# Dustin-Ray/capyCRYPT

Measured on NVIDIA B200. Metric: sha3_256_GBps, higher is better.
Workload: dtype u64

## Files before the change

### capycrypt_b200/csrc/keccak_bs.cuh

```cuda
#pragma once
#include <cstdint>

#include "keccak.cuh"

namespace capy {

static __device__ const uint2 KECCAK_RC_BITS[32] = {
    {0x50F4F1u, 0x0DB916u}, {0x000000u, 0x8C7F94u}, {0x000000u, 0x000000u}, {0x000000u, 0x327356u},
    {0x000000u, 0x000000u}, {0x000000u, 0x000000u}, {0x000000u, 0x000000u}, {0x000000u, 0xB5D4DEu},
    {0x000000u, 0x000000u}, {0x000000u, 0x000000u}, {0x000000u, 0x000000u}, {0x000000u, 0x000000u},
    {0x000000u, 0x000000u}, {0x000000u, 0x000000u}, {0x000000u, 0x000000u}, {0x000000u, 0xD81C68u},
    {0x000000u, 0x000000u}, {0x000000u, 0x000000u}, {0x000000u, 0x000000u}, {0x000000u, 0x000000u},
    {0x000000u, 0x000000u}, {0x000000u, 0x000000u}, {0x000000u, 0x000000u}, {0x000000u, 0x000000u},
    {0x000000u, 0x000000u}, {0x000000u, 0x000000u}, {0x000000u, 0x000000u}, {0x000000u, 0x000000u},
    {0x000000u, 0x000000u}, {0x000000u, 0x000000u}, {0x000000u, 0x000000u}, {0x000000u, 0xBBE0CCu}};

template <int K>
__device__ __forceinline__ uint32_t bs_from(uint32_t v, uint32_t lane) {
  if constexpr (K % 32 == 0) return v;
  else return __shfl_sync(0xffffffffu, v, (int)(lane - (uint32_t)K));
}

template <int R>
__device__ __forceinline__ void bs_rot(uint32_t (&b)[2], uint32_t t0, uint32_t t1, uint32_t lane) {
  if constexpr (R % 2 == 0) {
    b[0] = bs_from<R / 2>(t0, lane);
    b[1] = bs_from<R / 2>(t1, lane);
  } else {
    b[0] = bs_from<(R + 1) / 2>(t1, lane);
    b[1] = bs_from<(R - 1) / 2>(t0, lane);
  }
}

#define CAPY_BS_RHO_PI(X, Y, R)                                                                       \
  bs_rot<(R)>(b[(Y) + 5 * ((2 * (X) + 3 * (Y)) % 5)],                                                 \
              lop_xor3(a[(X) + 5 * (Y)][0], c[((X) + 4) % 5][0], n[((X) + 1) % 5][0]),                \
              lop_xor3(a[(X) + 5 * (Y)][1], c[((X) + 4) % 5][1], n[((X) + 1) % 5][1]), lane);

__device__ __forceinline__ uint32_t bs_flip_if(uint32_t v, uint32_t rounds, uint32_t round) {
  asm("{\n\t.reg .pred p;\n\t.reg .b32 t;\n\tand.b32 t, %1, %2;\n\tsetp.ne.u32 p, t, 0;\n\t@p not.b32 %0, %0;\n\t}"
      : "+r"(v)
      : "r"(rounds), "r"(round));
  return v;
}

__device__ __forceinline__ void keccak_bs_round(uint32_t (&a)[25][2], uint32_t lane, uint2 rc, uint32_t round) {
  uint32_t c[5][2], n[5][2], b[25][2];
#pragma unroll
  for (int x = 0; x < 5; x++) {
#pragma unroll
    for (int h = 0; h < 2; h++) c[x][h] = lop_xor3(lop_xor3(a[x][h], a[x + 5][h], a[x + 10][h]), a[x + 15][h], a[x + 20][h]);
    n[x][0] = bs_from<1>(c[x][1], lane);
    n[x][1] = c[x][0];
  }
  CAPY_BS_RHO_PI(0, 0, 0)  CAPY_BS_RHO_PI(1, 0, 1)  CAPY_BS_RHO_PI(2, 0, 62) CAPY_BS_RHO_PI(3, 0, 28) CAPY_BS_RHO_PI(4, 0, 27)
  CAPY_BS_RHO_PI(0, 1, 36) CAPY_BS_RHO_PI(1, 1, 44) CAPY_BS_RHO_PI(2, 1, 6)  CAPY_BS_RHO_PI(3, 1, 55) CAPY_BS_RHO_PI(4, 1, 20)
  CAPY_BS_RHO_PI(0, 2, 3)  CAPY_BS_RHO_PI(1, 2, 10) CAPY_BS_RHO_PI(2, 2, 43) CAPY_BS_RHO_PI(3, 2, 25) CAPY_BS_RHO_PI(4, 2, 39)
  CAPY_BS_RHO_PI(0, 3, 41) CAPY_BS_RHO_PI(1, 3, 45) CAPY_BS_RHO_PI(2, 3, 15) CAPY_BS_RHO_PI(3, 3, 21) CAPY_BS_RHO_PI(4, 3, 8)
  CAPY_BS_RHO_PI(0, 4, 18) CAPY_BS_RHO_PI(1, 4, 2)  CAPY_BS_RHO_PI(2, 4, 61) CAPY_BS_RHO_PI(3, 4, 56) CAPY_BS_RHO_PI(4, 4, 14)
#pragma unroll
  for (int y = 0; y < 5; y++) {
#pragma unroll
    for (int x = 0; x < 5; x++) {
#pragma unroll
      for (int h = 0; h < 2; h++)
        a[x + 5 * y][h] = lop_chi(b[x + 5 * y][h], b[(x + 1) % 5 + 5 * y][h], b[(x + 2) % 5 + 5 * y][h]);
    }
  }
  a[0][0] = bs_flip_if(a[0][0], rc.x, round);
  a[0][1] = bs_flip_if(a[0][1], rc.y, round);
}
#undef CAPY_BS_RHO_PI

struct BsTranspose {
  uint32_t rot[5], keep[5];
  __device__ __forceinline__ explicit BsTranspose(uint32_t lane) {
#pragma unroll
    for (int k = 0; k < 5; k++) {
      const uint32_t d = 16u >> k;
      const uint32_t lo_bits = k == 0 ? 0x0000FFFFu : k == 1 ? 0x00FF00FFu : k == 2 ? 0x0F0F0F0Fu : k == 3 ? 0x33333333u : 0x55555555u;
      const bool upper = lane & d;
      rot[k] = upper ? 32u - d : d;
      keep[k] = upper ? ~lo_bits : lo_bits;
    }
  }
  __device__ __forceinline__ uint32_t operator()(uint32_t x) const {
#pragma unroll
    for (int k = 0; k < 5; k++) {
      const uint32_t y = __shfl_xor_sync(0xffffffffu, x, 16u >> k);
      const uint32_t r = __funnelshift_l(y, y, rot[k]);
      asm("lop3.b32 %0, %0, %1, %2, 0xE4;" : "+r"(x) : "r"(r), "r"(keep[k]));
    }
    return x;
  }
};

__device__ __forceinline__ void bs_gather(uint32_t (&w)[2], uint32_t lo, uint32_t hi, uint32_t lane) {
#pragma unroll
  for (int h = 0; h < 2; h++) {
    const int src = (int)(2 * lane + h);
    const uint32_t l = __shfl_sync(0xffffffffu, lo, src);
    const uint32_t u = __shfl_sync(0xffffffffu, hi, src);
    w[h] = lane < 16 ? l : u;
  }
}

__device__ __forceinline__ void bs_scatter(uint32_t& lo, uint32_t& hi, const uint32_t (&w)[2], uint32_t lane) {
  const int src = (int)(lane >> 1);
  const uint32_t l0 = __shfl_sync(0xffffffffu, w[0], src), l1 = __shfl_sync(0xffffffffu, w[1], src);
  const uint32_t u0 = __shfl_sync(0xffffffffu, w[0], src + 16), u1 = __shfl_sync(0xffffffffu, w[1], src + 16);
  lo = lane & 1 ? l1 : l0;
  hi = lane & 1 ? u1 : u0;
}

}
```

### capycrypt_b200/csrc/sha3_api.cu

```cuda
#include <algorithm>
#include <cmath>
#include <cstdlib>
#include <memory>
#include <thread>
#include <type_traits>
#include <vector>

#include "internal.h"
#include "hostbatch.h"
#include "keccak_bs.cuh"
#include "sponge.cuh"

namespace capy {

template <int LANES>
__global__ void __launch_bounds__(128)
    sha3_uniform_kernel(const uint8_t* __restrict__ data, uint64_t stride, uint64_t len, uint32_t suffix,
                        uint8_t* __restrict__ out, uint32_t out_bytes, uint64_t n) {
  const uint64_t i = (uint64_t)blockIdx.x * blockDim.x + threadIdx.x;
  if (i >= n) return;
  constexpr uint64_t RATE = 8ull * LANES;
  const uint2* q = reinterpret_cast<const uint2*>(data + i * stride);
  Lane a[25];
  state_zero(a);
  const uint64_t nfull = len / RATE;
  for (uint64_t b = 0; b < nfull; b++) {
#pragma unroll
    for (int j = 0; j < LANES; j++) {
      uint2 v = __ldg(q + j);
      a[j].lo ^= v.x;
      a[j].hi ^= v.y;
    }
    q += LANES;
    keccak_f1600(a);
  }
  const uint32_t rem = (uint32_t)(len - nfull * RATE);
#pragma unroll
  for (int j = 0; j < LANES; j++) {
    const uint32_t o = 8u * j;
    uint32_t lo = 0, hi = 0;
    if (o < rem) {
      uint2 v = __ldg(q + j);
      lo = v.x;
      hi = v.y;
      if (o + 8 > rem) {
        const uint32_t keep = rem - o;
        if (keep < 4) {
          lo &= (1u << (8 * keep)) - 1u;
          hi = 0;
        } else if (keep > 4) {
          hi &= (1u << (8 * (keep - 4))) - 1u;
        } else {
          hi = 0;
        }
      }
    }
    if (rem >= o && rem < o + 8) {
      const uint32_t k = rem - o;
      if (k < 4) lo |= suffix << (8 * k);
      else hi |= suffix << (8 * (k - 4));
    }
    a[j].lo ^= lo;
    a[j].hi ^= hi;
  }
  if (rem + 1 < RATE) a[LANES - 1].hi ^= 0x80000000u;
  keccak_f1600(a);

  uint8_t* o = out + i * (uint64_t)out_bytes;
  if ((out_bytes & 15u) == 0 && (reinterpret_cast<uintptr_t>(out) & 15u) == 0) {
#pragma unroll
    for (int j = 0; j < 4; j++)
      if (16u * j < out_bytes)
        reinterpret_cast<uint4*>(o)[j] = make_uint4(a[2 * j].lo, a[2 * j].hi, a[2 * j + 1].lo, a[2 * j + 1].hi);
  } else {
#pragma unroll
    for (int j = 0; j < 8; j++) {
      if (8u * j < out_bytes) reinterpret_cast<uint32_t*>(o)[2 * j] = a[j].lo;
      if (8u * j + 4 < out_bytes) reinterpret_cast<uint32_t*>(o)[2 * j + 1] = a[j].hi;
    }
  }
}

template <int LANES, int MSG_LANES>
__global__ void __launch_bounds__(128, 4)
    sha3_short_kernel(const uint4* __restrict__ data, uint64_t stride16, uint32_t suffix, uint4* __restrict__ out,
                      uint32_t out_bytes, uint64_t n) {
  static_assert(MSG_LANES % 2 == 0 && MSG_LANES < LANES, "whole 16-byte loads, one block");
  constexpr int OUT_LANES = (200 - 8 * LANES) / 16;
  const uint32_t lane = threadIdx.x & 31u;
  const uint64_t i = (uint64_t)blockIdx.x * blockDim.x + threadIdx.x;
  if (i - lane >= n) return;
  const bool live = i < n;
  const BsTranspose transpose(lane);

  uint32_t a[25][2];
  {
    const uint4* q = data + i * stride16;
    uint32_t w[2 * MSG_LANES];
#pragma unroll
    for (int j = 0; j < MSG_LANES / 2; j++) {
      const uint4 v = live ? __ldg(q + j) : make_uint4(0u, 0u, 0u, 0u);
      w[4 * j] = v.x;
      w[4 * j + 1] = v.y;
      w[4 * j + 2] = v.z;
      w[4 * j + 3] = v.w;
    }
#pragma unroll
    for (int j = 0; j < 2 * MSG_LANES; j++) w[j] = transpose(w[j]);
#pragma unroll
    for (int l = 0; l < MSG_LANES; l++) bs_gather(a[l], w[2 * l], w[2 * l + 1], lane);
  }
#pragma unroll
  for (int l = MSG_LANES; l < 25; l++) a[l][0] = a[l][1] = 0u;
  const uint32_t pad = (uint32_t)((uint64_t)suffix >> (2 * lane));
  a[MSG_LANES][0] = 0u - (pad & 1u);
  a[MSG_LANES][1] = 0u - ((pad >> 1) & 1u);
  a[LANES - 1][1] ^= lane == 31 ? 0xFFFFFFFFu : 0u;

  const uint2 rc = __ldg(&KECCAK_RC_BITS[lane]);
  keccak_bs_round(a, lane, rc, 1u);
#pragma unroll 1
  for (int r = 1; r < 23; r += 2) {
    keccak_bs_round(a, lane, rc, 1u << r);
    keccak_bs_round(a, lane, rc, 2u << r);
  }
  keccak_bs_round(a, lane, rc, 1u << 23);

  uint32_t w[2 * OUT_LANES];
#pragma unroll
  for (int l = 0; l < OUT_LANES; l++) bs_scatter(w[2 * l], w[2 * l + 1], a[l], lane);
#pragma unroll
  for (int j = 0; j < 2 * OUT_LANES; j++) w[j] = transpose(w[j]);
  if (!live) return;
  uint4* o = out + i * (uint64_t)(out_bytes / 16);
#pragma unroll
  for (int j = 0; j < OUT_LANES / 2; j++) o[j] = make_uint4(w[4 * j], w[4 * j + 1], w[4 * j + 2], w[4 * j + 3]);
}

template <int LANES>
__global__ void prefix_state_kernel(const uint8_t* prefix, uint32_t nblocks, uint64_t* state) {
  if (threadIdx.x != 0 || blockIdx.x != 0) return;
  Lane a[25];
  state_zero(a);
  for (uint32_t b = 0; b < nblocks; b++) {
    const uint8_t* p = prefix + (size_t)b * 8 * LANES;
#pragma unroll
    for (int j = 0; j < LANES; j++) {
      uint64_t v = 0;
      for (int k = 0; k < 8; k++) v |= (uint64_t)p[8 * j + k] << (8 * k);
      a[j].lo ^= (uint32_t)v;
      a[j].hi ^= (uint32_t)(v >> 32);
    }
    keccak_f1600(a);
  }
  for (int k = 0; k < 25; k++) state[k] = ((uint64_t)a[k].hi << 32) | a[k].lo;
}

constexpr uint32_t kLenBins = 1u << 14;
constexpr uint64_t kHostPlanMaxItems = 1ull << 18;

__device__ __forceinline__ uint32_t len_bin(const uint64_t* off, uint64_t i, uint32_t stride_bytes) {
  const uint64_t blocks = (off[i + 1] - off[i]) / stride_bytes;
  return blocks < kLenBins - 1 ? (uint32_t)blocks : kLenBins - 1;
}

__global__ void len_hist_kernel(const uint64_t* __restrict__ off, uint64_t n, uint32_t stride_bytes, uint32_t* hist) {
  const uint64_t i = (uint64_t)blockIdx.x * blockDim.x + threadIdx.x;
  if (i < n) atomicAdd(&hist[len_bin(off, i, stride_bytes)], 1u);
}

__global__ void __launch_bounds__(1024) len_scan_kernel(uint32_t* hist, uint32_t* summary) {
  __shared__ unsigned long long tot_s;
  __shared__ uint32_t max_s, bins_s;
  const uint32_t t = threadIdx.x;
  constexpr uint32_t PER = kLenBins / 1024;
  static_assert(PER == 16, "four uint4 per thread");
  if (t == 0) { tot_s = 0; max_s = 0; bins_s = 0; }
  __syncthreads();
  const uint32_t lo = kLenBins - (t + 1) * PER;
  uint32_t c[PER];
#pragma unroll
  for (int q = 0; q < 4; q++) {
    const uint4 v = reinterpret_cast<const uint4*>(hist + lo)[q];
    c[4 * q] = v.x; c[4 * q + 1] = v.y; c[4 * q + 2] = v.z; c[4 * q + 3] = v.w;
  }
  uint32_t sum = 0, nb = 0, mx = 0;
  unsigned long long tot = 0;
#pragma unroll
  for (int k = 0; k < (int)PER; k++) {
    sum += c[k];
    if (c[k]) { nb++; mx = lo + k; }
    tot += (unsigned long long)c[k] * (lo + k + 1);
  }
  if (sum) {
    atomicAdd(&tot_s, tot);
    atomicMax(&max_s, mx);
    atomicAdd(&bins_s, nb);
  }
  __syncthreads();
  uint32_t incl = sum;
#pragma unroll
  for (int d = 1; d < 32; d <<= 1) {
    const uint32_t v = __shfl_up_sync(0xffffffffu, incl, d);
    if ((t & 31) >= (uint32_t)d) incl += v;
  }
  __shared__ uint32_t wsum[32];
  if ((t & 31) == 31) wsum[t >> 5] = incl;
  __syncthreads();
  if (t < 32) {
    uint32_t w = wsum[t];
#pragma unroll
    for (int d = 1; d < 32; d <<= 1) {
      const uint32_t v = __shfl_up_sync(0xffffffffu, w, d);
      if (t >= (uint32_t)d) w += v;
    }
    wsum[t] = w;
  }
  __syncthreads();
  uint32_t run = incl - sum + ((t >> 5) ? wsum[(t >> 5) - 1] : 0u);
#pragma unroll
  for (int k = (int)PER - 1; k >= 0; k--) {
    const uint32_t cnt = c[k];
    c[k] = run;
    run += cnt;
  }
#pragma unroll
  for (int q = 0; q < 4; q++) reinterpret_cast<uint4*>(hist + lo)[q] = make_uint4(c[4 * q], c[4 * q + 1], c[4 * q + 2], c[4 * q + 3]);
  if (t == 0) {
    summary[0] = (uint32_t)tot_s;
    summary[1] = (uint32_t)(tot_s >> 32);
    summary[2] = max_s;
    summary[3] = bins_s;
  }
}

__global__ void len_scatter_kernel(const uint64_t* __restrict__ off, uint64_t n, uint32_t stride_bytes, uint32_t* cursor,
                                   uint32_t* __restrict__ order) {
  const uint64_t i = (uint64_t)blockIdx.x * blockDim.x + threadIdx.x;
  if (i < n) order[atomicAdd(&cursor[len_bin(off, i, stride_bytes)], 1u)] = (uint32_t)i;
}

constexpr double kPairChainRatio = 3.08 / 4.6;
constexpr int kMaxWarpCosched = 3;
constexpr double kWarpChainRatio[kMaxWarpCosched + 1] = {0.0, 2.06 / 4.6, 2.36 / 4.6, 3.00 / 4.6};

static void plan_tiers(const std::vector<uint32_t>& cum, uint64_t n, uint32_t max_blocks, double total_blocks, int sm_count,
                       uint64_t warp_items[kMaxWarpCosched], uint64_t* pair_items, int force_c = 0) {
  for (int c = 0; c < kMaxWarpCosched; c++) warp_items[c] = 0;
  *pair_items = 0;
  const size_t nb = cum.size();
  std::vector<double> work_above(nb);
  double acc = 0;
  for (size_t k = nb; k-- > 0;) {
    work_above[k] = acc;
    const uint64_t cnt = (k == 0 ? n : cum[k - 1]) - cum[k];
    acc += (double)cnt * (double)(k + 1);
  }
  auto longer_than = [&](double thr, uint64_t* count, double* work) {
    if (thr < 1.0) {
      *count = n;
      *work = total_blocks;
      return;
    }
    const size_t k = std::min<size_t>((size_t)thr - 1, nb - 1);
    *count = cum[k];
    *work = work_above[k];
  };
  const double l1 = (double)max_blocks;
  const int c_first = force_c >= 1 && force_c <= kMaxWarpCosched ? force_c : 1;
  for (double T = l1 * kWarpChainRatio[c_first]; T < l1; T *= 1.01) {
    uint64_t k_above[kMaxWarpCosched + 2];
    double w_above[kMaxWarpCosched + 2];
    k_above[0] = 0;
    w_above[0] = 0;
    for (int c = 1; c <= kMaxWarpCosched; c++) {
      const int next = c + 1;
      const double ratio = next <= kMaxWarpCosched ? kWarpChainRatio[next] : kPairChainRatio;
      longer_than(T / ratio, &k_above[c], &w_above[c]);
      if (force_c && c != force_c) {
        k_above[c] = c < force_c ? 0 : k_above[force_c];
        w_above[c] = c < force_c ? 0 : w_above[force_c];
      }
    }
    uint64_t k_fast;
    double w_fast;
    longer_than(T, &k_fast, &w_fast);
    if (k_above[kMaxWarpCosched] == 0 && T < l1 * kPairChainRatio) continue;
    uint64_t blocks = 0;
    double sm_time = 0;
    uint64_t cnt[kMaxWarpCosched];
    for (int c = 1; c <= kMaxWarpCosched; c++) {
      cnt[c - 1] = k_above[c] - k_above[c - 1];
      blocks += (cnt[c - 1] + 4 * c - 1) / (4 * c);
      sm_time += (w_above[c] - w_above[c - 1]) * kWarpChainRatio[c] / (4.0 * c);
    }
    const uint64_t k_p = k_fast - k_above[kMaxWarpCosched];
    blocks += (k_p + 63) / 64;
    sm_time += (w_fast - w_above[kMaxWarpCosched]) * kPairChainRatio / 64.0 + (total_blocks - w_fast) / 128.0;
    if (blocks + 1 > (uint64_t)sm_count) continue;
    if (sm_time > 0.95 * T * (double)sm_count) continue;
    if ((total_blocks - w_fast) / 128.0 > T * (double)((uint64_t)sm_count - blocks)) continue;
    for (int c = 0; c < kMaxWarpCosched; c++) warp_items[c] = cnt[c];
    *pair_items = k_p;
    return;
  }
}

template <int... Ls, class F>
static int with_lanes(int lanes, F&& f) {
  int rc = CAPY_ERR_BAD_ARG;
  (void)((lanes == Ls && ((rc = f(std::integral_constant<int, Ls>())), true)) || ...);
  return rc;
}

struct CudaFree {
  void operator()(void* p) const { cudaFree(p); }
};
template <class T>
using DevPtr = std::unique_ptr<T, CudaFree>;
template <class T>
static cudaError_t dev_alloc(DevPtr<T>& p, size_t bytes) {
  T* q = nullptr;
  const cudaError_t e = cudaMalloc(&q, bytes);
  if (e == cudaSuccess) p.reset(q);
  return e;
}

struct LenHist {
  uint64_t total_blocks = 0;
  uint32_t max_bin = 0;
  uint32_t bins = 0;
  std::vector<uint32_t> cnt;
};

static void host_len_hist(const uint64_t* h_off, uint64_t n, uint32_t stride_bytes, LenHist* h) {
  h->cnt.assign(kLenBins, 0);
  const double inv = 1.0 / (double)stride_bytes;
  for (uint64_t i = 0; i < n; i++) {
    const uint64_t len = h_off[i + 1] - h_off[i];
    uint64_t q = (uint64_t)((double)len * inv);
    if (q * stride_bytes > len) q--;
    else if ((q + 1) * stride_bytes <= len) q++;
    const uint32_t b = q < kLenBins - 1 ? (uint32_t)q : kLenBins - 1;
    if (h->cnt[b]++ == 0) h->bins++;
    if (b > h->max_bin) h->max_bin = b;
    h->total_blocks += (uint64_t)b + 1;
  }
}

static int device_len_hist(capy_ctx* ctx, cudaStream_t st, const uint64_t* d_off, uint64_t n, uint32_t stride_bytes,
                           uint32_t* hist, LenHist* h) {
  uint32_t* summary = hist + kLenBins;
  CAPY_CUDA(ctx, cudaMemsetAsync(hist, 0, (size_t)kLenBins * 4 + 64, st));
  len_hist_kernel<<<(unsigned)((n + 255) / 256), 256, 0, st>>>(d_off, n, stride_bytes, hist);
  len_scan_kernel<<<1, 1024, 0, st>>>(hist, summary);
  ctx->launches += 2;
  if (!h->cnt.empty()) return CAPY_OK;
  uint32_t h_sum[4];
  CAPY_CUDA(ctx, cudaMemcpyAsync(h_sum, summary, sizeof h_sum, cudaMemcpyDeviceToHost, st));
  CAPY_CUDA(ctx, cudaStreamSynchronize(st));
  h->total_blocks = (uint64_t)h_sum[0] | ((uint64_t)h_sum[1] << 32);
  h->max_bin = h_sum[2];
  h->bins = h_sum[3];
  return CAPY_OK;
}

static int plan_from_hist(capy_ctx* ctx, DeviceCtx& dc, cudaStream_t st, const uint64_t* d_off, uint64_t n,
                          uint32_t stride_bytes, const LenHist& h, uint32_t* hist, uint32_t* order, bool allow_pair,
                          int force_c, LaunchPlan* plan) {
  const uint32_t max_blocks = h.max_bin + 1;
  const double ideal = (double)h.total_blocks / (32.0 * 4.0 * dc.sm_count);
  if (allow_pair && max_blocks > 64 && (double)max_blocks > 1.05 * ideal) {
    std::vector<uint32_t> cum(kLenBins);
    if (!h.cnt.empty()) {
      uint32_t above = 0;
      for (uint32_t k = kLenBins; k-- > 0;) {
        cum[k] = above;
        above += h.cnt[k];
      }
    } else {
      CAPY_CUDA(ctx, cudaMemcpyAsync(cum.data(), hist, (size_t)kLenBins * 4, cudaMemcpyDeviceToHost, st));
      CAPY_CUDA(ctx, cudaStreamSynchronize(st));
    }
    plan_tiers(cum, n, max_blocks, (double)h.total_blocks, dc.sm_count, plan->warp_items, &plan->pair_items, force_c);
  }
  if (h.bins == 1) plan->uniform_blocks = max_blocks;
  if (h.bins > 1) {
    len_scatter_kernel<<<(unsigned)((n + 255) / 256), 256, 0, st>>>(d_off, n, stride_bytes, hist, order);
    ctx->launches++;
    CAPY_CUDA(ctx, cudaGetLastError());
    plan->order = order;
    plan->warps_per_smsp = 0;
    if ((double)max_blocks * 4.0 > 0.7 * ideal) {
      plan->warps_per_smsp = 3;
      if ((double)max_blocks * 3.0 > 0.7 * ideal) plan->warps_per_smsp = 2;
      if ((double)max_blocks * 2.0 > 0.7 * ideal) plan->warps_per_smsp = 1;
    }
  }
  return CAPY_OK;
}

static int plan_ragged(capy_ctx* ctx, DeviceCtx& dc, cudaStream_t st, const uint64_t* d_off, uint64_t n,
                       uint32_t stride_bytes, LaunchPlan* plan, bool allow_pair = true, int force_c = 0) {
  *plan = LaunchPlan();
  if (n < 1 || n > 0xffffffffull) return CAPY_OK;
  const uint64_t* h_off = host_off_find(dc, d_off, n);
  LenHist h;
  if (h_off) {
    const uint64_t len0 = h_off[1] - h_off[0];
    bool uniform = true;
    for (uint64_t i = 1; i < n && uniform; i++) uniform = (h_off[i + 1] - h_off[i]) == len0;
    if (uniform) {
      plan->uniform_blocks = len0 / stride_bytes + 1;
      return CAPY_OK;
    }
    if (n > kHostPlanMaxItems) h_off = nullptr;
    else host_len_hist(h_off, n, stride_bytes, &h);
  }
  const bool cached = ctx->plan_cache.load() != 0 && force_c == 0 && !h_off;
  if (cached) {
    for (PlanEntry& e : dc.plans)
      if (e.off == d_off && e.n == n && e.unit == stride_bytes && e.allow_pair == allow_pair) {
        e.last_use = ++dc.use_clock;
        *plan = e.plan;
        return CAPY_OK;
      }
  }
  uint32_t* hist = (uint32_t*)scratch_get(dc, st, kPlanHist, (size_t)kLenBins * 4 + 64);
  DevPtr<uint32_t> owned;
  if (cached && dev_alloc(owned, (size_t)n * 4) != cudaSuccess) {
    cudaGetLastError();
    return CAPY_ERR_OOM;
  }
  uint32_t* order = cached ? owned.get() : (uint32_t*)scratch_get(dc, st, kPlanOrder, (size_t)n * 4);
  if (!hist || !order) return CAPY_ERR_OOM;
  int rc = device_len_hist(ctx, st, d_off, n, stride_bytes, hist, &h);
  if (rc) return rc;
  rc = plan_from_hist(ctx, dc, st, d_off, n, stride_bytes, h, hist, order, allow_pair, force_c, plan);
  if (rc) return rc;
  if (cached) {
    if (!plan->order) owned.reset();
    if (dc.plans.size() >= kMaxPlanEntries) {
      size_t lru = 0;
      for (size_t k = 1; k < dc.plans.size(); k++)
        if (dc.plans[k].last_use < dc.plans[lru].last_use) lru = k;
      if (dc.plans[lru].owned_order) cudaFree(dc.plans[lru].owned_order);
      dc.plans.erase(dc.plans.begin() + lru);
    }
    PlanEntry e;
    e.off = d_off;
    e.n = n;
    e.unit = stride_bytes;
    e.allow_pair = allow_pair;
    e.plan = *plan;
    e.owned_order = owned.release();
    e.last_use = ++dc.use_clock;
    dc.plans.push_back(e);
  }
  return CAPY_OK;
}

template <class Kernel>
static cudaError_t throttle(Kernel* kernel, const LaunchPlan& plan, unsigned* block, size_t* smem) {
  *smem = 0;
  if (plan.warps_per_smsp < 1 || plan.warps_per_smsp > 3) return cudaSuccess;
  *block = 128;
  *smem = (size_t)(227 * 1024 / plan.warps_per_smsp) - 1024;
  return cudaFuncSetAttribute(kernel, cudaFuncAttributeMaxDynamicSharedMemorySize, 226 * 1024);
}

template <int LANES>
static int launch_sponge_t(capy_ctx* ctx, cudaStream_t stream, SpongeJob J, unsigned block, const LaunchPlan& plan) {
  if (plan.tiered()) {
    const uint64_t warp_items = plan.warp_items[0] + plan.warp_items[1] + plan.warp_items[2], pair_items = plan.pair_items;
    SpongeTiers tiers;
    uint32_t warp_blocks = 0;
    uint64_t rank = 0;
    for (int c = 0; c < 3; c++) {
      tiers.first_block[c] = warp_blocks;
      tiers.first_rank[c] = rank;
      warp_blocks += grid_for(plan.warp_items[c], 4 * (c + 1));
      rank += plan.warp_items[c];
    }
    tiers.warp_blocks = warp_blocks;
    tiers.pair_blocks = grid_for(2 * pair_items, 128);
    const unsigned solo_blocks = grid_for(J.n - pair_items - warp_items, 128);
    J.warp_items = warp_items;
    J.first = warp_items + pair_items;
    CAPY_CUDA(ctx, cudaFuncSetAttribute(sponge_tiered_kernel<LANES>, cudaFuncAttributeMaxDynamicSharedMemorySize, 226 * 1024));
    sponge_tiered_kernel<LANES><<<warp_blocks + tiers.pair_blocks + solo_blocks, 384, 226 * 1024, stream>>>(J, tiers);
    ctx->launches++;
    CAPY_CUDA(ctx, cudaGetLastError());
    return CAPY_OK;
  }
  size_t smem;
  CAPY_CUDA(ctx, throttle(sponge_kernel<LANES>, plan, &block, &smem));
  sponge_kernel<LANES><<<grid_for(J.n, block), block, smem, stream>>>(J);
  ctx->launches++;
  CAPY_CUDA(ctx, cudaGetLastError());
  return CAPY_OK;
}

static unsigned pick_block(uint64_t n, int sm_count, int threads_per_sm) {
  unsigned best = 128;
  double best_eff = -1.0;
  for (unsigned bs : {128u, 64u, 32u}) {
    const uint64_t blocks = (n + bs - 1) / bs;
    const uint64_t slots = (uint64_t)sm_count * (threads_per_sm / bs);
    const uint64_t waves = (blocks + slots - 1) / slots;
    const double per_sm = (double)blocks / sm_count;
    const double busiest = waves > 1 ? (double)waves * (threads_per_sm / bs) : (double)((blocks + sm_count - 1) / sm_count);
    const double eff = per_sm / busiest;
    if (eff > best_eff + 0.02) {
      best_eff = eff;
      best = bs;
    }
  }
  return best;
}

static int job_lanes(const SpongeJob& J) { return (int)(J.rate / 8); }

static int launch_sponge(capy_ctx* ctx, DeviceCtx& dc, cudaStream_t stream, const SpongeJob& J, const LaunchPlan& plan) {
  if (J.n == 0) return CAPY_OK;
  const unsigned block = pick_block(J.n, dc.sm_count, 384);
  return with_lanes<9, 13, 17, 18, 19, 21>(job_lanes(J), [&](auto L) {
    return launch_sponge_t<decltype(L)::value>(ctx, stream, J, block, plan);
  });
}

static int launch_sponge_seq(capy_ctx* ctx, DeviceCtx& dc, cudaStream_t stream, const SpongeJob& A, const SpongeJob& B,
                             const LaunchPlan& plan) {
  const int rc = launch_sponge(ctx, dc, stream, A, plan);
  if (rc) return rc;
  return launch_sponge(ctx, dc, stream, B, plan);
}

static bool chain_jobs_fit(int sm_count, uint64_t n) {
  if (getenv("CAPY_NO_CHAIN_SPLIT") || sm_count < 1) return false;
  return (n + 127) / 128 >= (uint64_t)CAPY_SPONGE_MINB * (uint64_t)sm_count;
}

static bool chain_cut(int sm_count, uint64_t n, uint64_t absorb_blocks, uint64_t squeeze_extra, uint64_t* cut) {
  if (!chain_jobs_fit(sm_count, n)) return false;
  const uint64_t warps = (n + 31) / 32, sched = 4ull * (uint64_t)sm_count;
  if (warps > 8 * sched) return false;
  auto fill = [&](uint64_t w) {
    const double x = (double)w / (double)sched;
    return x / std::ceil(x);
  };
  if (fill(2 * warps) < fill(warps) + 0.04) return false;
  const uint64_t perms = absorb_blocks + squeeze_extra;
  if (perms < 12) return false;
  uint64_t k = (perms + 1) / 2;
  if (k > absorb_blocks) k = absorb_blocks;
  if (3 * k < perms) return false;
  *cut = k;
  return true;
}

static int launch_chain_jobs(capy_ctx* ctx, DeviceCtx& dc, cudaStream_t stream, const SpongeJob& J0, const SpongeJob& J1,
                             bool data_dependent, uint32_t jobs = 2, const SpongeResume* resume = nullptr) {
  const uint32_t nb = (uint32_t)((J0.n + 127) / 128);
  uint32_t* sync = (uint32_t*)scratch_get(dc, stream, kChainSync, ((size_t)nb + 1) * sizeof(uint32_t));
  if (!sync) return CAPY_ERR_OOM;
  CAPY_CUDA(ctx, cudaMemsetAsync(sync, 0, ((size_t)nb + 1) * sizeof(uint32_t), stream));
  SpongeChain C;
  C.j[0] = J0;
  C.j[1] = J1;
  C.sync = sync;
  C.blocks_per_job = nb;
  C.data_dependent = data_dependent ? 1u : 0u;
  C.resume = resume ? *resume : SpongeResume{};
  return with_lanes<9, 13, 17, 18, 19, 21>(job_lanes(J0), [&](auto L) {
    sponge_chain_kernel<decltype(L)::value><<<jobs * nb, 128, 0, stream>>>(C);
    ctx->launches++;
    CAPY_CUDA(ctx, cudaGetLastError());
    return CAPY_OK;
  });
}

static int launch_sponge_chain(capy_ctx* ctx, DeviceCtx& dc, cudaStream_t stream, const SpongeJob& J, uint64_t cut) {
  uint64_t* states = (uint64_t*)scratch_get(dc, stream, kChainStates, (size_t)J.n * 25 * sizeof(uint64_t));
  if (!states) return CAPY_ERR_OOM;
  SpongeJob J0 = J, J1 = J;
  J0.chain_out = states;
  J0.stop_block = J.skip_blocks + cut;
  J1.chain_in = states;
  J1.skip_blocks = (uint32_t)(J.skip_blocks + cut);
  return launch_chain_jobs(ctx, dc, stream, J0, J1, false);
}

static bool uniform_cut(const DeviceCtx& dc, const SpongeJob& J, const LaunchPlan& plan, uint64_t* cut) {
  if (J.out_off || J.xor_in || plan.order || (J.rate & 7u) != 0) return false;
  const uint64_t msg_blocks = J.off ? plan.uniform_blocks : J.msg_len / J.rate + 1;
  if (!msg_blocks) return false;
  uint64_t absorb = msg_blocks;
  if (J.keys) absorb += ((uint64_t)J.key_len + 8) / J.w + 1;
  if (!J.skip_blocks) absorb += J.prefix_len / J.rate;
  const uint64_t sq = 8ull * J.sq_lanes, squeeze_extra = J.out_bytes ? (J.out_bytes + sq - 1) / sq - 1 : 0;
  return chain_cut(dc.sm_count, J.n, absorb, squeeze_extra, cut);
}

static int run_sponge(capy_ctx* ctx, DeviceCtx& dc, cudaStream_t stream, SpongeJob J, const LaunchPlan& plan) {
  J.order = plan.order;
  uint64_t cut;
  if (uniform_cut(dc, J, plan, &cut)) return launch_sponge_chain(ctx, dc, stream, J, cut);
  return launch_sponge(ctx, dc, stream, J, plan);
}

static int launch_sha3(capy_ctx* ctx, DeviceCtx& dc, cudaStream_t stream, int d, const uint8_t* data, const uint64_t* off,
                       uint64_t msg_len, uint64_t stride, uint64_t n, uint8_t* out, uint32_t flags = 0,
                       bool tail_readable = true) {
  if (!valid_secparam(d)) return CAPY_ERR_BAD_SECPARAM;
  if (n == 0) return CAPY_OK;
  if (!off && !tail_readable && (msg_len & 7u) != 0 && n > 1 && (reinterpret_cast<uintptr_t>(data) & 7u) == 0 &&
      (stride & 7u) == 0 && (reinterpret_cast<uintptr_t>(out) & 3u) == 0) {
    int rc = launch_sha3(ctx, dc, stream, d, data, nullptr, msg_len, stride, n - 1, out, flags, true);
    if (rc) return rc;
    return launch_sha3(ctx, dc, stream, d, data + (n - 1) * stride, nullptr, msg_len, stride, 1, out + (n - 1) * (uint64_t)(d / 8),
                       flags, false);
  }
  const uint32_t rate = (1600 - sha3_capacity(d)) / 8;
  const int lanes = (int)rate / 8;
  if (!off && (reinterpret_cast<uintptr_t>(data) & 15u) == 0 && (reinterpret_cast<uintptr_t>(out) & 15u) == 0 &&
      (stride & 15u) == 0 && (d == 256 || d == 512) && msg_len >= 16 && (msg_len & 15u) == 0 && msg_len < rate) {
    const unsigned block = 128, grid = grid_for(n, block);
    const uint4* dq = reinterpret_cast<const uint4*>(data);
    uint4* oq = reinterpret_cast<uint4*>(out);
    const uint64_t s16 = stride / 16;
    const int msg_lanes = (int)(msg_len / 8);
    const int rc = d == 256 ? with_lanes<2, 4, 6, 8, 10, 12, 14, 16>(msg_lanes, [&](auto M) {
      sha3_short_kernel<17, decltype(M)::value><<<grid, block, 0, stream>>>(dq, s16, 0x06u, oq, 32, n);
      return CAPY_OK;
    }) : with_lanes<2, 4, 6, 8>(msg_lanes, [&](auto M) {
      sha3_short_kernel<9, decltype(M)::value><<<grid, block, 0, stream>>>(dq, s16, 0x06u, oq, 64, n);
      return CAPY_OK;
    });
    if (rc) return rc;
    ctx->launches++;
    CAPY_CUDA(ctx, cudaGetLastError());
    return CAPY_OK;
  }
  SpongeJob J{};
  J.data = data;
  J.off = off;
  J.msg_len = msg_len;
  J.msg_stride = stride;
  J.trailer_len = 1;
  J.sha3_suffix = 1;
  J.rate = rate;
  J.out = out;
  J.out_stride = J.out_bytes = (uint64_t)d / 8;
  J.sq_lanes = (1600 - d) / 64;
  J.n = n;
  uint64_t cut;
  if (!off && !uniform_cut(dc, J, LaunchPlan(), &cut) && (reinterpret_cast<uintptr_t>(data) & 7u) == 0 &&
      (stride & 7u) == 0 && (reinterpret_cast<uintptr_t>(out) & 3u) == 0 && (tail_readable || (msg_len & 7u) == 0)) {
    const uint32_t suffix = (msg_len % 136u == 135u) ? 0x86u : 0x06u;
    const unsigned block = 128, grid = grid_for(n, block);
    return with_lanes<9, 13, 17, 18>(lanes, [&](auto L) {
      sha3_uniform_kernel<decltype(L)::value><<<grid, block, 0, stream>>>(data, stride, msg_len, suffix, out, d / 8, n);
      ctx->launches++;
      CAPY_CUDA(ctx, cudaGetLastError());
      return CAPY_OK;
    });
  }
  LaunchPlan plan;
  if (off && !(flags & CAPY_FLAG_NO_SORT)) {
    int rc = plan_ragged(ctx, dc, stream, off, n, rate, &plan, !(flags & CAPY_FLAG_NO_PAIR),
                         (int)((flags >> CAPY_FLAG_WARP_COSCHED_SHIFT) & 3u));
    if (rc) return rc;
  }
  return run_sponge(ctx, dc, stream, J, plan);
}

static void host_left_encode(std::string& o, uint64_t v) {
  if (v == 0) {
    o.push_back(1);
    o.push_back(0);
    return;
  }
  int nb = 8;
  while (nb > 1 && ((v >> (8 * (nb - 1))) & 0xFF) == 0) nb--;
  o.push_back((char)nb);
  for (int i = nb - 1; i >= 0; i--) o.push_back((char)((v >> (8 * i)) & 0xFF));
}
static void host_encode_string(std::string& o, const uint8_t* s, size_t n) {
  host_left_encode(o, (uint64_t)n * 8);
  o.append(reinterpret_cast<const char*>(s), n);
}

static int get_prefix(capy_ctx* ctx, DeviceCtx& dc, cudaStream_t stream, int d, const uint8_t* fn, uint32_t fn_len,
                      const uint8_t* cs, uint32_t cs_len, PrefixState** out) {
  std::string key;
  key.push_back((char)(d >> 8));
  key.push_back((char)d);
  host_left_encode(key, fn_len);
  key.append(reinterpret_cast<const char*>(fn), fn_len);
  key.append(reinterpret_cast<const char*>(cs), cs_len);
  auto it = dc.prefix_cache.find(key);
  if (it != dc.prefix_cache.end()) {
    it->second.last_use = ++dc.use_clock;
    *out = &it->second;
    return CAPY_OK;
  }
  if (dc.prefix_cache.size() >= kMaxPrefixEntries) {
    auto lru = dc.prefix_cache.begin();
    for (auto k = dc.prefix_cache.begin(); k != dc.prefix_cache.end(); ++k)
      if (k->second.last_use < lru->second.last_use) lru = k;
    if (lru->second.d_state) cudaFree(lru->second.d_state);
    if (lru->second.d_prefix) cudaFree(lru->second.d_prefix);
    dc.prefix_cache.erase(lru);
  }
  const uint32_t w = bytepad_value(d);
  std::string p;
  host_left_encode(p, w);
  host_encode_string(p, fn, fn_len);
  host_encode_string(p, cs, cs_len);
  p.append(w - p.size() % w, '\0');
  PrefixState ps;
  ps.prefix_len = (uint32_t)p.size();
  DevPtr<uint8_t> d_prefix;
  DevPtr<uint64_t> d_state;
  CAPY_CUDA(ctx, dev_alloc(d_prefix, p.size()));
  CAPY_CUDA(ctx, dev_alloc(d_state, 25 * sizeof(uint64_t)));
  CAPY_CUDA(ctx, cudaMemcpyAsync(d_prefix.get(), p.data(), p.size(), cudaMemcpyHostToDevice, stream));
  if (w % 8 == 0) {
    ps.skip_blocks = ps.prefix_len / w;
    const int rc = with_lanes<17, 19, 21>((int)(w / 8), [&](auto L) {
      prefix_state_kernel<decltype(L)::value><<<1, 32, 0, stream>>>(d_prefix.get(), ps.skip_blocks, d_state.get());
      ctx->launches++;
      CAPY_CUDA(ctx, cudaGetLastError());
      return CAPY_OK;
    });
    if (rc) return rc;
  } else {
    ps.skip_blocks = 0;
  }
  CAPY_CUDA(ctx, cudaStreamSynchronize(stream));
  ps.d_prefix = d_prefix.release();
  ps.d_state = d_state.release();
  ps.last_use = ++dc.use_clock;
  auto ins = dc.prefix_cache.emplace(key, ps);
  *out = &ins.first->second;
  return CAPY_OK;
}

static void fill_cshake_common(SpongeJob& J, int d, const PrefixState* ps) {
  const uint32_t w = bytepad_value(d);
  J.prefix = ps->d_prefix;
  J.prefix_len = ps->prefix_len;
  J.init_state = ps->skip_blocks ? ps->d_state : nullptr;
  J.skip_blocks = ps->skip_blocks;
  J.w = w;
  J.rate = (1600 - d) / 8;
  J.sq_lanes = (1600 - d) / 64;
}

static int launch_cshake(capy_ctx* ctx, DeviceCtx& dc, cudaStream_t stream, int d, const uint8_t* data,
                         const uint64_t* off, uint64_t n, const uint8_t* fn, uint32_t fn_len, const uint8_t* cs,
                         uint32_t cs_len, uint64_t out_bits, uint8_t* out) {
  if (!valid_secparam(d)) return CAPY_ERR_BAD_SECPARAM;
  if (n == 0 || out_bits / 8 == 0) return CAPY_OK;
  PrefixState* ps;
  int rc = get_prefix(ctx, dc, stream, d, fn, fn_len, cs, cs_len, &ps);
  if (rc) return rc;
  SpongeJob J{};
  fill_cshake_common(J, d, ps);
  J.data = data;
  J.off = off;
  J.trailer = 0x04;
  J.trailer_len = 1;
  if (fn_len == 0 && cs_len == 0) J.q4_rate = (1600 - sha3_capacity(d)) / 8;
  J.out = out;
  J.out_stride = J.out_bytes = out_bits / 8;
  J.n = n;
  LaunchPlan plan;
  rc = plan_ragged(ctx, dc, stream, off, n, J.rate & ~7u, &plan);
  if (rc) return rc;
  return run_sponge(ctx, dc, stream, J, plan);
}

static int build_kmac_job(capy_ctx* ctx, DeviceCtx& dc, cudaStream_t stream, const KmacDevArgs& a, SpongeJob* out) {
  static const uint8_t kKmac[4] = {'K', 'M', 'A', 'C'};
  PrefixState* ps;
  int rc = get_prefix(ctx, dc, stream, a.d_bits, kKmac, 4, a.custom, a.custom_len, &ps);
  if (rc) return rc;
  SpongeJob J{};
  fill_cshake_common(J, a.d_bits, ps);
  J.keys = a.keys;
  J.key_off = a.key_off;
  J.key_len = (uint32_t)a.key_len;
  J.key_stride = a.key_stride;
  J.data = a.data;
  J.off = a.off;
  J.msg_len = a.msg_len;
  J.msg_stride = a.msg_stride;
  J.trailer = 0x040100u;
  J.trailer_len = 3;
  J.out = a.out;
  J.out_off = a.out_off;
  J.out_stride = a.out_stride;
  J.out_bytes = a.out_bytes;
  J.xor_in = a.xor_in;
  J.n = a.n;
  *out = J;
  return CAPY_OK;
}

static int plan_kmac(capy_ctx* ctx, DeviceCtx& dc, cudaStream_t stream, const KmacDevArgs& a, const SpongeJob& J, LaunchPlan* plan) {
  *plan = LaunchPlan();
  if (a.no_sort) return CAPY_OK;
  if (a.off) return plan_ragged(ctx, dc, stream, a.off, a.n, J.rate & ~7u, plan);
  if (a.out_off) return plan_ragged(ctx, dc, stream, a.out_off, a.n, 8u * J.sq_lanes, plan);
  return CAPY_OK;
}

int launch_kmac_xof(capy_ctx* ctx, DeviceCtx& dc, cudaStream_t stream, const KmacDevArgs& a) {
  if (!valid_secparam(a.d_bits)) return CAPY_ERR_BAD_SECPARAM;
  if (a.n == 0) return CAPY_OK;
  if (!a.out_off && a.out_bytes == 0) return CAPY_OK;
  SpongeJob J;
  int rc = build_kmac_job(ctx, dc, stream, a, &J);
  if (rc) return rc;
  LaunchPlan plan;
  rc = plan_kmac(ctx, dc, stream, a, J, &plan);
  if (rc) return rc;
  return run_sponge(ctx, dc, stream, J, plan);
}

template <int LANES>
static int launch_sponge2_t(capy_ctx* ctx, cudaStream_t stream, const SpongeJob& A, const SpongeJob& B, unsigned block,
                            const LaunchPlan& plan) {
  SpongeJob2 JJ;
  JJ.j[0] = A;
  JJ.j[1] = B;
  size_t smem;
  CAPY_CUDA(ctx, throttle(sponge_kernel2<LANES>, plan, &block, &smem));
  const uint64_t warps = 2 * ((A.n + 31) / 32);
  sponge_kernel2<LANES><<<grid_for(warps * 32, block), block, smem, stream>>>(JJ);
  ctx->launches++;
  CAPY_CUDA(ctx, cudaGetLastError());
  return CAPY_OK;
}

int launch_kmac_xof2(capy_ctx* ctx, DeviceCtx& dc, cudaStream_t stream, const KmacDevArgs& a, const KmacDevArgs& b) {
  if (!valid_secparam(a.d_bits) || a.d_bits != b.d_bits || a.n != b.n) return CAPY_ERR_BAD_ARG;
  if (a.n == 0) return CAPY_OK;
  SpongeJob JA, JB;
  int rc = build_kmac_job(ctx, dc, stream, a, &JA);
  if (rc) return rc;
  rc = build_kmac_job(ctx, dc, stream, b, &JB);
  if (rc) return rc;
  LaunchPlan plan;
  rc = plan_kmac(ctx, dc, stream, a, JA, &plan);
  if (rc) return rc;
  JA.order = JB.order = plan.order;
  if (plan.tiered()) return launch_sponge_seq(ctx, dc, stream, JA, JB, plan);
  const unsigned block = pick_block(2 * a.n, dc.sm_count, 384);
  return with_lanes<17, 19, 21>(job_lanes(JA), [&](auto L) {
    return launch_sponge2_t<decltype(L)::value>(ctx, stream, JA, JB, block, plan);
  });
}

int launch_kmac_xof_dep(capy_ctx* ctx, DeviceCtx& dc, cudaStream_t stream, const KmacDevArgs& first, const KmacDevArgs& second) {
  if (!valid_secparam(first.d_bits) || first.d_bits != second.d_bits || first.n != second.n) return CAPY_ERR_BAD_ARG;
  if (first.n == 0) return CAPY_OK;
  SpongeJob J0, J1;
  int rc = build_kmac_job(ctx, dc, stream, first, &J0);
  if (rc) return rc;
  rc = build_kmac_job(ctx, dc, stream, second, &J1);
  if (rc) return rc;
  LaunchPlan plan;
  rc = plan_kmac(ctx, dc, stream, second, J1, &plan);
  if (rc) return rc;
  J0.order = J1.order = plan.order;
  if (plan.tiered() || (J0.rate & 7u) != 0 || !chain_jobs_fit(dc.sm_count, first.n))
    return launch_sponge_seq(ctx, dc, stream, J0, J1, plan);
  return launch_chain_jobs(ctx, dc, stream, J0, J1, true);
}

static int hasher_check(const capy_ctx* ctx, const capy_hasher* h) { return h && ctx && h->ctx == ctx ? CAPY_OK : CAPY_ERR_BAD_ARG; }
static uint64_t hasher_items(const capy_hasher* h, int k) { return h->first[k + 1] - h->first[k]; }
static bool hasher_any_finished(const capy_hasher* h) {
  for (char f : h->finished)
    if (f) return true;
  return false;
}
static std::vector<Range> hasher_shards(const capy_hasher* h) {
  std::vector<Range> s;
  for (size_t k = 0; k + 1 < h->first.size(); k++) s.push_back({h->first[k], h->first[k + 1]});
  return s;
}

static SpongeJob hasher_job(const capy_hasher* h, int k, uint64_t j0, uint64_t n, SpongeResume* R) {
  SpongeJob J{};
  J.rate = h->rate;
  J.sq_lanes = (1600 - h->d_bits) / 64;
  if (h->kmac) {
    J.trailer = 0x040100u;
    J.trailer_len = 3;
  } else {
    J.sha3_suffix = 1;
    J.trailer_len = 1;
  }
  J.chain_in = h->d_state[k] + j0;
  J.n = n;
  R->carry = h->d_carry[k] + j0 * h->rate;
  R->totals = h->d_total[k] + j0;
  R->state_n = hasher_items(h, k);
  return J;
}

static int hasher_update_items(capy_ctx* ctx, DeviceCtx& dc, cudaStream_t st, capy_hasher* h, uint64_t j0, uint64_t n,
                               const uint8_t* d_data, const uint64_t* d_off) {
  if (n == 0) return CAPY_OK;
  SpongeResume R;
  SpongeJob J = hasher_job(h, dc.index, j0, n, &R);
  J.chain_out = h->d_state[dc.index] + j0;
  J.stop_block = ~0ull;
  J.data = d_data;
  J.off = d_off;
  return launch_chain_jobs(ctx, dc, st, J, J, false, 1, &R);
}

static int hasher_final_items(capy_ctx* ctx, DeviceCtx& dc, cudaStream_t st, const capy_hasher* h, uint64_t j0, uint64_t n,
                              uint64_t out_bytes, const uint64_t* d_out_off, uint8_t* d_out) {
  if (n == 0 || (!d_out_off && out_bytes == 0)) return CAPY_OK;
  SpongeResume R;
// ... 443 lines not shown
```

### profiles/extract_sass.py

```python
import collections
import glob
import os
import re
import subprocess

ROOT = os.path.dirname(os.path.dirname(os.path.abspath(__file__)))
OBJ = sorted(glob.glob(os.path.join(ROOT, "capycrypt_b200", "_lib", "obj_*")), key=os.path.getmtime)[-1]
OUT = os.path.join(ROOT, "profiles", "sass")
os.makedirs(OUT, exist_ok=True)


def functions(obj):
    txt = subprocess.run(["cuobjdump", "-sass", obj], capture_output=True, text=True).stdout
    res = {}
    for part in re.split(r"\n\s+Function : ", txt)[1:]:
        name, body = part.split("\n", 1)
        ins = []
        for line in body.split("\n"):
            m = re.match(r"\s+/\*([0-9a-f]{4,5})\*/\s+(.*?);", line)
            if m:
                ins.append((int(m.group(1), 16), m.group(2).strip()))
        res[name.strip()] = ins
    return res


def opcode(t):
    t = re.sub(r"^@!?U?P\d+\s+", "", t)
    op = t.split()[0]
    base = op.split(".")[0]
    if base == "IMAD" and ".WIDE" in op:
        return "IMAD.WIDE"
    return base


def loops(ins):
    addr = {a: i for i, (a, _) in enumerate(ins)}
    for i, (a, t) in enumerate(ins):
        if re.match(r"(@!?U?P\d+\s+)?BRA", t):
            m = re.search(r"0x([0-9a-f]+)", t)
            if m and int(m.group(1), 16) < a and int(m.group(1), 16) in addr:
                yield addr[int(m.group(1), 16)], i


def dump(path, header, ins):
    with open(path, "w") as f:
        f.write("// " + header + "\n")
        for a, t in ins:
            f.write(f"/*{a:05x}*/  {t} ;\n")


sha3 = functions(os.path.join(OBJ, "sha3_api.o"))
var = functions(os.path.join(OBJ, "ed448_var.o"))
hist = []
for name, ins in list(sha3.items()) + list(functions(os.path.join(OBJ, "ed448_fixed.o")).items()) + list(var.items()):
    c = collections.Counter(opcode(t) for _, t in ins)
    hist.append(f"{name[:90]}\n    {len(ins)} instructions: " + ", ".join(f"{k} {v}" for k, v in c.most_common(12)))
open(os.path.join(OUT, "opcode_histograms.txt"), "w").write("\n".join(hist) + "\n")

short = next(v for k, v in sha3.items() if "sha3_short_kernelILi17ELi8E" in k)
s, e = max(loops(short), key=lambda se: se[1] - se[0])
dump(os.path.join(OUT, "keccak_round_x2.sass"), "sha3_short_kernel<17, 8>: loop body = two Keccak-f rounds", short[s:e + 1])

tier = next(v for k, v in sha3.items() if "sponge_tiered_kernelILi9E" in k)
bfly = [i for i, (_, t) in enumerate(tier) if "SHFL.BFLY" in t]
cands = [(s, e) for s, e in loops(tier) if s <= bfly[0] <= e]
s, e = min(cands, key=lambda se: se[1] - se[0])
dump(os.path.join(OUT, "keccak_pair_round.sass"), "sponge_tiered_kernel<9>, pair tier: loop body = four rounds of the split-lane permutation", tier[s:e + 1])
idx = [i for i, (_, t) in enumerate(tier) if "SHFL.IDX PT" in t]
dump(os.path.join(OUT, "keccak_warp_round.sass"), "sponge_tiered_kernel<9>, warp tier: first two rounds of the unrolled one-lane-per-thread permutation",
     tier[idx[0] - 6: idx[36] + 12])

first_bfly = bfly[0]
ldg = [i for i, (_, t) in enumerate(tier) if "LDG.E.CONSTANT" in t and i < first_bfly]
dump(os.path.join(OUT, "pair_prefetch_before_permutation.sass"),
     "sponge_tiered_kernel<9>, pair tier: predicated loads of the next block, then the first instructions of the permutation",
     tier[max(0, ldg[-1] - 24): first_bfly + 4])

chain = next(v for k, v in sha3.items() if "sponge_chain_kernelILi17E" in k)
ns = [i for i, (_, t) in enumerate(chain) if "NANOSLEEP" in t]
at = [i for i, (_, t) in enumerate(chain) if t.split()[0].startswith(("ATOM", "RED")) or " ATOM" in t or " RED" in t]
if ns:
    dump(os.path.join(OUT, "chain_ticket_and_wait.sass"),
         "sponge_chain_kernel<17>: ticket (ATOM), job / block from the ticket, job 1 waiting for the job-0 block of its items",
         chain[max(0, at[0] - 6): ns[-1] + 10])
if len(at) > 1:
    dump(os.path.join(OUT, "chain_report.sass"), "sponge_chain_kernel<17>: a job-0 warp reports (fence, RED) after storing its states",
         chain[max(0, at[-1] - 40): at[-1] + 3])

vb = next(v for k, v in var.items() if "var_base_kernel" in k)
calls = collections.Counter(re.search(r"0x([0-9a-f]+)", t).group(1) for _, t in vb if t.startswith("CALL"))
rets = [i for i, (_, t) in enumerate(vb) if t.startswith("RET")]
for tgt, _ in calls.most_common():
    a0 = int(tgt, 16)
    i0 = next(i for i, (a, _) in enumerate(vb) if a == a0)
    i1 = next(r for r in rets if r >= i0)
    body = vb[i0:i1 + 1]
    wide = sum(1 for _, t in body if "IMAD.WIDE" in t)
    if wide > 150:
        dump(os.path.join(OUT, "fe_mul.sass"), f"fe_mul_call (ed448_var.cu): {len(body)} instructions, {wide} IMAD.WIDE", body)
    elif wide > 90:
        dump(os.path.join(OUT, "fe_sqr.sass"), f"fe_sqr_call (ed448_var.cu): {len(body)} instructions, {wide} IMAD.WIDE", body)
print(sorted(os.listdir(OUT)))
```

Baseline: 310.4.

## Process two bitsliced message groups per warp in short SHA3 kernel

Each warp now hashes two independent groups of 32 messages, interleaving one Keccak round of each so the shuffle-heavy bitsliced rounds have more independent work to hide shuffle latency. The grid is halved to match, and the iota flip is simplified into a precomputed predicate struct shared by both groups. The unroll-by-two of rounds is replaced by a one-round loop body covering both groups. Register pressure roughly doubles, so the launch bound drops from 4 to 3 blocks per SM, which lowers occupancy.

```diff
diff --git a/capycrypt_b200/csrc/keccak_bs.cuh b/capycrypt_b200/csrc/keccak_bs.cuh
--- a/capycrypt_b200/csrc/keccak_bs.cuh
+++ b/capycrypt_b200/csrc/keccak_bs.cuh
@@ -37,14 +37,12 @@
               lop_xor3(a[(X) + 5 * (Y)][0], c[((X) + 4) % 5][0], n[((X) + 1) % 5][0]),                \
               lop_xor3(a[(X) + 5 * (Y)][1], c[((X) + 4) % 5][1], n[((X) + 1) % 5][1]), lane);
 
-__device__ __forceinline__ uint32_t bs_flip_if(uint32_t v, uint32_t rounds, uint32_t round) {
-  asm("{\n\t.reg .pred p;\n\t.reg .b32 t;\n\tand.b32 t, %1, %2;\n\tsetp.ne.u32 p, t, 0;\n\t@p not.b32 %0, %0;\n\t}"
-      : "+r"(v)
-      : "r"(rounds), "r"(round));
-  return v;
-}
+struct BsIota {
+  bool x, y;
+  __device__ __forceinline__ BsIota(uint2 rc, uint32_t round) : x((rc.x & round) != 0u), y((rc.y & round) != 0u) {}
+};
 
-__device__ __forceinline__ void keccak_bs_round(uint32_t (&a)[25][2], uint32_t lane, uint2 rc, uint32_t round) {
+__device__ __forceinline__ void keccak_bs_round(uint32_t (&a)[25][2], uint32_t lane, BsIota iota) {
   uint32_t c[5][2], n[5][2], b[25][2];
 #pragma unroll
   for (int x = 0; x < 5; x++) {
@@ -67,8 +65,8 @@
         a[x + 5 * y][h] = lop_chi(b[x + 5 * y][h], b[(x + 1) % 5 + 5 * y][h], b[(x + 2) % 5 + 5 * y][h]);
     }
   }
-  a[0][0] = bs_flip_if(a[0][0], rc.x, round);
-  a[0][1] = bs_flip_if(a[0][1], rc.y, round);
+  if (iota.x) a[0][0] = ~a[0][0];
+  if (iota.y) a[0][1] = ~a[0][1];
 }
 #undef CAPY_BS_RHO_PI
 
diff --git a/capycrypt_b200/csrc/sha3_api.cu b/capycrypt_b200/csrc/sha3_api.cu
--- a/capycrypt_b200/csrc/sha3_api.cu
+++ b/capycrypt_b200/csrc/sha3_api.cu
@@ -82,59 +82,86 @@
 }
 
 template <int LANES, int MSG_LANES>
-__global__ void __launch_bounds__(128, 4)
+__device__ __forceinline__ void bs_load_block(uint32_t (&a)[25][2], uint32_t (&w)[2 * MSG_LANES], const BsTranspose& transpose,
+                                              uint32_t suffix, uint32_t lane) {
+#pragma unroll
+  for (int j = 0; j < 2 * MSG_LANES; j++) w[j] = transpose(w[j]);
+#pragma unroll
+  for (int l = 0; l < MSG_LANES; l++) bs_gather(a[l], w[2 * l], w[2 * l + 1], lane);
+#pragma unroll
+  for (int l = MSG_LANES; l < 25; l++) a[l][0] = a[l][1] = 0u;
+  const uint32_t pad = (uint32_t)((uint64_t)suffix >> (2 * lane));
+  a[MSG_LANES][0] = 0u - (pad & 1u);
+  a[MSG_LANES][1] = 0u - ((pad >> 1) & 1u);
+  a[LANES - 1][1] ^= lane == 31 ? 0xFFFFFFFFu : 0u;
+}
+
+template <int OUT_LANES>
+__device__ __forceinline__ void bs_store_digest(uint32_t (&w)[2 * OUT_LANES], const uint32_t (&a)[25][2], const BsTranspose& transpose,
+                                                uint32_t lane) {
+#pragma unroll
+  for (int l = 0; l < OUT_LANES; l++) bs_scatter(w[2 * l], w[2 * l + 1], a[l], lane);
+#pragma unroll
+  for (int j = 0; j < 2 * OUT_LANES; j++) w[j] = transpose(w[j]);
+}
+
+template <int LANES, int MSG_LANES>
+__global__ void __launch_bounds__(128, 3)
     sha3_short_kernel(const uint4* __restrict__ data, uint64_t stride16, uint32_t suffix, uint4* __restrict__ out,
                       uint32_t out_bytes, uint64_t n) {
   static_assert(MSG_LANES % 2 == 0 && MSG_LANES < LANES, "whole 16-byte loads, one block");
   constexpr int OUT_LANES = (200 - 8 * LANES) / 16;
   const uint32_t lane = threadIdx.x & 31u;
-  const uint64_t i = (uint64_t)blockIdx.x * blockDim.x + threadIdx.x;
-  if (i - lane >= n) return;
-  const bool live = i < n;
+  const uint64_t i0 = 2 * ((uint64_t)blockIdx.x * blockDim.x + threadIdx.x) - lane, i1 = i0 + 32;
+  if (i0 - lane >= n) return;
+  const bool live0 = i0 < n, live1 = i1 < n;
+
+  uint32_t w0[2 * MSG_LANES], w1[2 * MSG_LANES];
+  {
+    const uint4* q0 = data + i0 * stride16;
+    const uint4* q1 = data + i1 * stride16;
+#pragma unroll
+    for (int j = 0; j < MSG_LANES / 2; j++) {
+      const uint4 v0 = live0 ? __ldg(q0 + j) : make_uint4(0u, 0u, 0u, 0u);
+      const uint4 v1 = live1 ? __ldg(q1 + j) : make_uint4(0u, 0u, 0u, 0u);
+      w0[4 * j] = v0.x, w0[4 * j + 1] = v0.y, w0[4 * j + 2] = v0.z, w0[4 * j + 3] = v0.w;
+      w1[4 * j] = v1.x, w1[4 * j + 1] = v1.y, w1[4 * j + 2] = v1.z, w1[4 * j + 3] = v1.w;
+    }
+  }
   const BsTranspose transpose(lane);
-
-  uint32_t a[25][2];
+  const uint2 rc = __ldg(&KECCAK_RC_BITS[lane]);
+  uint32_t a0[25][2], a1[25][2];
+  bs_load_block<LANES, MSG_LANES>(a0, w0, transpose, suffix, lane);
+  bs_load_block<LANES, MSG_LANES>(a1, w1, transpose, suffix, lane);
   {
-    const uint4* q = data + i * stride16;
-    uint32_t w[2 * MSG_LANES];
-#pragma unroll
-    for (int j = 0; j < MSG_LANES / 2; j++) {
-      const uint4 v = live ? __ldg(q + j) : make_uint4(0u, 0u, 0u, 0u);
-      w[4 * j] = v.x;
-      w[4 * j + 1] = v.y;
-      w[4 * j + 2] = v.z;
-      w[4 * j + 3] = v.w;
-    }
-#pragma unroll
-    for (int j = 0; j < 2 * MSG_LANES; j++) w[j] = transpose(w[j]);
-#pragma unroll
-    for (int l = 0; l < MSG_LANES; l++) bs_gather(a[l], w[2 * l], w[2 * l + 1], lane);
-  }
-#pragma unroll
-  for (int l = MSG_LANES; l < 25; l++) a[l][0] = a[l][1] = 0u;
-  const uint32_t pad = (uint32_t)((uint64_t)suffix >> (2 * lane));
-  a[MSG_LANES][0] = 0u - (pad & 1u);
-  a[MSG_LANES][1] = 0u - ((pad >> 1) & 1u);
-  a[LANES - 1][1] ^= lane == 31 ? 0xFFFFFFFFu : 0u;
-
-  const uint2 rc = __ldg(&KECCAK_RC_BITS[lane]);
-  keccak_bs_round(a, lane, rc, 1u);
+    const BsIota iota(rc, 1u);
+    keccak_bs_round(a0, lane, iota);
+    keccak_bs_round(a1, lane, iota);
+  }
 #pragma unroll 1
-  for (int r = 1; r < 23; r += 2) {
-    keccak_bs_round(a, lane, rc, 1u << r);
-    keccak_bs_round(a, lane, rc, 2u << r);
-  }
-  keccak_bs_round(a, lane, rc, 1u << 23);
-
-  uint32_t w[2 * OUT_LANES];
-#pragma unroll
-  for (int l = 0; l < OUT_LANES; l++) bs_scatter(w[2 * l], w[2 * l + 1], a[l], lane);
-#pragma unroll
-  for (int j = 0; j < 2 * OUT_LANES; j++) w[j] = transpose(w[j]);
-  if (!live) return;
-  uint4* o = out + i * (uint64_t)(out_bytes / 16);
-#pragma unroll
-  for (int j = 0; j < OUT_LANES / 2; j++) o[j] = make_uint4(w[4 * j], w[4 * j + 1], w[4 * j + 2], w[4 * j + 3]);
+  for (int r = 1; r < 23; r++) {
+    const BsIota iota(rc, 1u << r);
+    keccak_bs_round(a0, lane, iota);
+    keccak_bs_round(a1, lane, iota);
+  }
+  {
+    const BsIota iota(rc, 1u << 23);
+    keccak_bs_round(a0, lane, iota);
+    keccak_bs_round(a1, lane, iota);
+  }
+  uint32_t o0[2 * OUT_LANES], o1[2 * OUT_LANES];
+  bs_store_digest<OUT_LANES>(o0, a0, transpose, lane);
+  bs_store_digest<OUT_LANES>(o1, a1, transpose, lane);
+  uint4* p0 = out + i0 * (uint64_t)(out_bytes / 16);
+  uint4* p1 = out + i1 * (uint64_t)(out_bytes / 16);
+  if (live0) {
+#pragma unroll
+    for (int j = 0; j < OUT_LANES / 2; j++) p0[j] = make_uint4(o0[4 * j], o0[4 * j + 1], o0[4 * j + 2], o0[4 * j + 3]);
+  }
+  if (live1) {
+#pragma unroll
+    for (int j = 0; j < OUT_LANES / 2; j++) p1[j] = make_uint4(o1[4 * j], o1[4 * j + 1], o1[4 * j + 2], o1[4 * j + 3]);
+  }
 }
 
 template <int LANES>
@@ -625,7 +652,7 @@
   const int lanes = (int)rate / 8;
   if (!off && (reinterpret_cast<uintptr_t>(data) & 15u) == 0 && (reinterpret_cast<uintptr_t>(out) & 15u) == 0 &&
       (stride & 15u) == 0 && (d == 256 || d == 512) && msg_len >= 16 && (msg_len & 15u) == 0 && msg_len < rate) {
-    const unsigned block = 128, grid = grid_for(n, block);
+    const unsigned block = 128, grid = grid_for(32 * ((n + 63) / 64), block);
     const uint4* dq = reinterpret_cast<const uint4*>(data);
     uint4* oq = reinterpret_cast<uint4*>(out);
     const uint64_t s16 = stride / 16;
diff --git a/profiles/extract_sass.py b/profiles/extract_sass.py
--- a/profiles/extract_sass.py
+++ b/profiles/extract_sass.py
@@ -59,7 +59,7 @@
 
 short = next(v for k, v in sha3.items() if "sha3_short_kernelILi17ELi8E" in k)
 s, e = max(loops(short), key=lambda se: se[1] - se[0])
-dump(os.path.join(OUT, "keccak_round_x2.sass"), "sha3_short_kernel<17, 8>: loop body = two Keccak-f rounds", short[s:e + 1])
+dump(os.path.join(OUT, "keccak_round_x2.sass"), "sha3_short_kernel<17, 8>: loop body = one Keccak-f round of each of the two message groups", short[s:e + 1])
 
 tier = next(v for k, v in sha3.items() if "sponge_tiered_kernelILi9E" in k)
 bfly = [i for i, (_, t) in enumerate(tier) if "SHFL.BFLY" in t]
```

New measurement: 316.8 (median of 6 runs). 2.1% higher.
